# angela000/DQNFlappyBird

Measured on AMD Instinct MI355X. Metric: env steps/sec (whole node) + DQN grad-steps/sec, 80x80x4 batch=32, higher is better.
Workload: dtype f32

## Files before the change

### dqnflappybird_amd/csrc/fb_qnet.hip

```cpp
#include <math.h>
#include <stdlib.h>
#include "fb_common.h"

#ifndef FK_ABL
#define FK_ABL 0
#endif
#ifndef BW_ABL
#define BW_ABL 0
#endif

namespace {

typedef float f32x16 __attribute__((ext_vector_type(16)));

constexpr int OFF_W1 = 0, OFF_B1 = 8192, OFF_W2 = 8224, OFF_B2 = 40992, OFF_W3 = 41056, OFF_B3 = 77920,
              OFF_WF1 = 77984;
constexpr int CONV_PARAMS = OFF_WF1;
#include "fb_head.h"
#include "fb_sampler.h"
#include "fb_gather.h"
constexpr int MAXTB = 256;


struct Slice { const float *params; const uint8_t *states; int s_off, count; const uint16_t *w1s; int fshift; };
// ... 811 lines not shown
                const int Pp = tile * 8 + 2 * g + hl;
                if (Pp < 100) {
                    if (blockIdx.y == 0) { const size_t o = (row * 100 + Pp) * 32 + j; a.p1o[o] = bv; a.amax[o] = (uint8_t)best; }
                    uint16_t *d = reinterpret_cast<uint16_t *>(smem + Pp * 4 + (((j >> 3) + (Pp >> 2)) & 3)) + (j & 7);
                    if constexpr (NS == 3) {
                        const _Float16 hh = (_Float16)bv, ll = (_Float16)((bv - (float)hh) * F16_LO_SCALE);
                        d[0] = __builtin_bit_cast(uint16_t, hh); d[IN_P * 8] = __builtin_bit_cast(uint16_t, ll);
                        bad |= bv >= FB_F16_RANGE;
                    } else d[0] = (uint16_t)f32_to_bf16_rn(bv);
                }
            }
        }
    }
    __syncthreads();
    if (W16 && wave >= 8) { if constexpr (NS == 3) note_overflow(bad, a.ovf); return; }
    if (RING && C23T_EXIT == 2) { if (smem[tid].x == 0x12345u) a.h2[0] = 1.f; return; }
    const int oy = j / 5, ox = j - oy * 5;
    const bool rowok = j < 25;
    f32x16 acc = {0}, acl = {0};
    auto finish = [&](const float *__restrict__ bias, float *__restrict__ out, bool planes) {
#pragma unroll
        for (int r = 0; r < 16; r++) red[((kq * 2 + ct) * 16 + r) * 64 + lane] = NS == 3 ? fmaf(acl[r], F16_LO_UNSCALE, acc[r]) : acc[r];
        __syncthreads();
        const int ctp = wave & 1, q = wave >> 1;
        float v[4];
#pragma unroll
        for (int e = 0; e < 4; e++) {
            v[e] = red[((0 * 2 + ctp) * 16 + 4 * q + e) * 64 + lane];
#pragma unroll
            for (int k = 1; k < 4; k++) v[e] += red[((k * 2 + ctp) * 16 + 4 * q + e) * 64 + lane];
        }
        const int ch = ctp * 32 + 8 * q + 4 * hl;
        const float4 bv = *reinterpret_cast<const float4 *>(bias + ch);
        v[0] = fmaxf(v[0] + bv.x, 0.f); v[1] = fmaxf(v[1] + bv.y, 0.f); v[2] = fmaxf(v[2] + bv.z, 0.f); v[3] = fmaxf(v[3] + bv.w, 0.f);
        if (rowok) *reinterpret_cast<float4 *>(out + (row * 25 + j) * 64 + ch) = make_float4(v[0], v[1], v[2], v[3]);
        if ((planes || a.a3s) && rowok) {
            uint32_t h0, l0, h1, l1, m_;
            if constexpr (NS == 3) { split2x2(v[0], v[1], h0, l0); split2x2(v[2], v[3], h1, l1); bad |= out_of_f16_range(v[0], v[1], v[2], v[3]); }
            else { split3x2(v[0], v[1], h0, m_, l0); split3x2(v[2], v[3], h1, m_, l1); }
            if (planes) {
                uint2 *d = reinterpret_cast<uint2 *>(smem + C2O + j * 8 + ((ctp * 4 + q) ^ ((j >> 1) & 7))) + hl;
                d[0] = make_uint2(h0, h1);
                if (NS == 3) d[2 * C2_P] = make_uint2(l0, l1);
            } else {
                uint16_t *d = a.a3s + (row * 25 + j) * 64 + ch;
                *reinterpret_cast<uint2 *>(d) = make_uint2(h0, h1);
                if (NS == 3) *reinterpret_cast<uint2 *>(d + a.pl3) = make_uint2(l0, l1);
            }
        }
#pragma unroll
        for (int r = 0; r < 16; r++) { acc[r] = 0.f; acl[r] = 0.f; }
    };
#pragma unroll
    for (int c = 0; c < 17; c++) {
        int aidx[2];
        if (c < 8) {
            const int tap = 2 * c + (kq >> 1), iy = 2 * oy + (tap >> 2) - 1, ix = 2 * ox + (tap & 3) - 1, pix = iy * 10 + ix;
            const bool ok = rowok && iy >= 0 && iy < 10 && ix >= 0 && ix < 10;
#pragma unroll
            for (int p = 0; p < NPL; p++) aidx[p] = ok ? p * IN_P + pix * 4 + ((((kq & 1) * 2 + hl) + (pix >> 2)) & 3) : ZOFF;
        } else {
            const int tap = c - 8, ky = tap / 3, iy = oy + ky - 1, ix = ox + (tap - 3 * ky) - 1, pix = iy * 5 + ix;
            const bool ok = rowok && iy >= 0 && iy < 5 && ix >= 0 && ix < 5;
#pragma unroll
            for (int p = 0; p < NPL; p++) aidx[p] = ok ? C2O + p * C2_P + pix * 8 + ((2 * kq + hl) ^ ((pix >> 1) & 7)) : ZOFF;
        }
        uint4 A[NPL];
#pragma unroll
        for (int p = 0; p < NPL; p++) A[p] = smem[aidx[p]];
        const WF W = w0;
        w0 = w1; w1 = w2;
        if (c + 3 < 17) w2 = loadW(c + 3);
        if constexpr (NS == 3) {
            acl = mfma_h(W.v[0], A[1], acl);
            acl = mfma_h(W.v[1], A[0], acl);
            acc = mfma_h(W.v[0], A[0], acc);
        } else acc = mfma_b(W.v[0], A[0], acc);
        if (c == 7) { finish(s.params + OFF_B2, a.h2, true); __syncthreads(); }
    }
    finish(s.params + OFF_B3, a.h3, false);
    if constexpr (NS == 3) note_overflow(bad, a.ovf);
}

constexpr int FC1_SP_KS = 4;
struct Fc1Args { const uint16_t *ain; size_t aplane; const uint16_t *zeros; const uint4 *w; float *hfp; int stot, M, N;
                 const unsigned *pver; unsigned *wver;
                 const uint4 *w2; int m_split;
                 const float *hp_src; float *hp_dst; int hp_n;
                 unsigned long long *set_flag; unsigned long long set_val; };

#ifndef FC1_ABL
#define FC1_ABL 0
#endif
template <int NS>
__global__ __launch_bounds__(256) void fc1_sp_kernel(Fc1Args a) {
    constexpr int NPL = NS == 3 ? 2 : 1, P0 = NS == 3 ? 0 : 2;
    constexpr int ASZ = NPL * 512, BSZ = 4 * NPL * 64, SLOT = ASZ + BSZ;
    __shared__ uint4 smem[3 * SLOT];
    const int lane = threadIdx.x & 63, wave = threadIdx.x >> 6, hl = lane >> 5, j = lane & 31;
    if (a.wver && blockIdx.x == 0 && threadIdx.x == 0) *a.wver = *a.pver;
    if (a.hp_dst) { const int i = blockIdx.x * 256 + threadIdx.x; if (i < a.hp_n) a.hp_dst[i] = a.hp_src[i]; }
    if (a.set_flag && blockIdx.x == 0 && threadIdx.x == 0) fb_flag_store(a.set_flag, a.set_val);
    const int xcd = blockIdx.x & 7, w = blockIdx.x >> 3, nth = a.N >> 7;
    const int ks = xcd & 3, m0 = (w / nth) * 128, n0 = ((xcd >> 2) * nth + w % nth) * 64;
    const int cbase = ks * 12 + (ks < 2 ? ks : 2), count = ks < 2 ? 13 : 12;
    struct St { uint4 a0, a1, a2, a3, b0, b1; };
    const int r0 = min(m0 + (int)(threadIdx.x >> 2), a.M - 1), r1 = min(m0 + 64 + (int)(threadIdx.x >> 2), a.M - 1);
    const uint16_t *pa0 = a.ain + (size_t)r0 * 1600 + (size_t)cbase * 32 + (threadIdx.x & 3) * 8;
    const uint16_t *pa1 = a.ain + (size_t)r1 * 1600 + (size_t)cbase * 32 + (threadIdx.x & 3) * 8;
    auto ldA = [&](int c, int p, int i) { return *reinterpret_cast<const uint4 *>((i ? pa1 : pa0) + p * a.aplane + c * 32); };
    const uint4 *wsel = a.w2 && m0 >= a.m_split ? a.w2 : a.w;
    auto pbq = [&](int q) {
        const int e = wave + 4 * q, k8 = e / NPL, pl = e - k8 * NPL;
        return wsel + ((size_t)(cbase * 4 + k8) * 3 + P0 + pl) * a.N + n0 + lane;
    };
    const uint4 *pb0 = pbq(0), *pb1 = pbq(NPL == 2 ? 1 : 0);
    const size_t bstep = (size_t)12 * a.N;
    auto ldB = [&](int c, int q) {
        (void)c;
        const uint4 *&pb = q == 0 ? pb0 : pb1;
        const uint4 v = *pb;
        pb += bstep;
        return v;
    };
    auto load = [&](int c) {
        St r;
        r.a0 = ldA(c, 0, 0); r.a1 = ldA(c, 0, 1); r.b0 = ldB(c, 0);
        if (NPL == 2) { r.a2 = ldA(c, 1, 0); r.a3 = ldA(c, 1, 1); r.b1 = ldB(c, 1); }
        else { r.a2 = r.a0; r.a3 = r.a0; r.b1 = r.b0; }
        return r;
    };
    auto stA_ = [&](int slot, int p, int i, const uint4 v) {
        const int q = threadIdx.x + 256 * i, row = q >> 2;
        smem[slot * SLOT + p * 512 + row * 4 + ((q + (row >> 2)) & 3)] = v;
    };
    auto store = [&](int slot, const St r) {
        stA_(slot, 0, 0, r.a0); stA_(slot, 0, 1, r.a1);
        uint4 *d = smem + slot * SLOT + ASZ + wave * 64 + lane;
        d[0] = r.b0;
        if (NPL == 2) { stA_(slot, 1, 0, r.a2); stA_(slot, 1, 1, r.a3); d[256] = r.b1; }
    };
    struct Fr { uint4 A[NPL]; uint4 W[2][NPL]; };
    const int row = wave * 32 + j;
    auto readF = [&](int slot, int s) {
        Fr f;
#pragma unroll
        for (int p = 0; p < NPL; p++) {
            f.A[p] = smem[slot * SLOT + p * 512 + row * 4 + ((2 * s + hl + (row >> 2)) & 3)];
#pragma unroll
            for (int ct = 0; ct < 2; ct++) f.W[ct][p] = smem[slot * SLOT + ASZ + ((2 * s + hl) * NPL + p) * 64 + ct * 32 + j];
        }
        return f;
    };
    f32x16 acc[2] = {{0}, {0}}, acl[2] = {{0}, {0}};
    auto compute = [&](const Fr f) {
        if (FC1_ABL == 2) { acc[0][0] += __uint_as_float(f.A[0].x ^ f.W[0][0].y ^ f.W[1][NPL - 1].z ^ f.A[NPL - 1].w); return; }
#pragma unroll
        for (int ct = 0; ct < 2; ct++) {
            if constexpr (NS == 3) {
                acl[ct] = mfma_h(f.A[1], f.W[ct][0], acl[ct]);
                acl[ct] = mfma_h(f.A[0], f.W[ct][1], acl[ct]);
                acc[ct] = mfma_h(f.A[0], f.W[ct][0], acc[ct]);
            } else acc[ct] = mfma_b(f.A[0], f.W[ct][0], acc[ct]);
        }
    };
    St stA = load(0), stB = load(1);
// ... 2817 lines not shown
        FB_CHECK_HIP(hipMemsetD32Async((hipDeviceptr_t)(h->params[which] + h->sac_off.bq1), (int)bits, (size_t)h->A, fb_stream(stream)));
        FB_CHECK_HIP(hipMemsetD32Async((hipDeviceptr_t)(h->params[which] + h->sac_off.bq2), (int)bits, (size_t)h->A, fb_stream(stream)));
    }
    if (is_iqn(h)) {
        const float b = 1.0f;
        uint32_t bits;
        memcpy(&bits, &b, 4);
        FB_CHECK_HIP(hipMemsetD32Async((hipDeviceptr_t)(h->params[which] + h->iqn_off.be), (int)bits, (size_t)h->FC, fb_stream(stream)));
    }
    if (h->noisy)
        hipLaunchKernelGGL(noisy_sigma_init_kernel, dim3((unsigned)((h->n - OFF_WF1 + 255) / 256)), dim3(256), 0, fb_stream(stream), h->mst[which], h->nnet);
    noisy_materialise(h, which, 0, false, fb_stream(stream));
    env_noise_invalidate(h, which, fb_stream(stream));
    c51d_fold(h, which, fb_stream(stream));
    hipLaunchKernelGGL(w1_split_kernel, dim3(32), dim3(256), 0, fb_stream(stream), h->params[which], h->w1s[which], &h->adam->pver[which]);
    resplit_now(h, which, fb_stream(stream));
    FB_LAUNCH_CHECK();
    return FB_OK;
}

extern "C" int fb_qnet_load_params(fb_qnet_t h, int which, const float *flat, void *stream) {
    FB_REQUIRE(h && flat && (which == 0 || which == 1), "fb_qnet_load_params: bad argument");
    FB_CHECK_HIP(hipMemcpyAsync(master(h, which), flat, sizeof(float) * (size_t)h->ntot, hipMemcpyDeviceToDevice, fb_stream(stream)));
    noisy_materialise(h, which, 0, false, fb_stream(stream));
    env_noise_invalidate(h, which, fb_stream(stream));
    hipLaunchKernelGGL(w1_split_kernel, dim3(32), dim3(256), 0, fb_stream(stream), h->params[which], h->w1s[which], &h->adam->pver[which]);
    c51d_fold(h, which, fb_stream(stream));
    resplit_now(h, which, fb_stream(stream));
    FB_LAUNCH_CHECK();
    return FB_OK;
}

extern "C" int fb_qnet_store_params(fb_qnet_t h, int which, float *flat, void *stream) {
    FB_REQUIRE(h && flat && (which == 0 || which == 1), "fb_qnet_store_params: bad argument");
    FB_CHECK_HIP(hipMemcpyAsync(flat, master(h, which), sizeof(float) * (size_t)h->ntot, hipMemcpyDeviceToDevice, fb_stream(stream)));
    return FB_OK;
}

extern "C" int fb_qnet_get_adam_state(fb_qnet_t h, float *m, float *v, float *beta_pows_host) {
    FB_REQUIRE(h, "fb_qnet_get_adam_state: NULL handle");
    FB_CHECK_HIP(hipDeviceSynchronize());
    const size_t nb = sizeof(float) * (size_t)h->ntot;
    if (m) FB_CHECK_HIP(hipMemcpy(m, h->adam_m, nb, hipMemcpyDeviceToDevice));
    if (v) FB_CHECK_HIP(hipMemcpy(v, h->adam_v, nb, hipMemcpyDeviceToDevice));
    if (beta_pows_host) {
        AdamDev a;
        FB_CHECK_HIP(hipMemcpy(&a, h->adam, sizeof(a), hipMemcpyDeviceToHost));
        beta_pows_host[0] = a.b1pow; beta_pows_host[1] = a.b2pow;
    }
    return FB_OK;
}

extern "C" int fb_qnet_set_adam_state(fb_qnet_t h, const float *m, const float *v, const float *beta_pows_host) {
    FB_REQUIRE(h, "fb_qnet_set_adam_state: NULL handle");
    FB_CHECK_HIP(hipDeviceSynchronize());
    const size_t nb = sizeof(float) * (size_t)h->ntot;
    if (m) FB_CHECK_HIP(hipMemcpy(h->adam_m, m, nb, hipMemcpyDeviceToDevice));
    if (v) FB_CHECK_HIP(hipMemcpy(h->adam_v, v, nb, hipMemcpyDeviceToDevice));
    if (beta_pows_host) {
        AdamDev a;
        FB_CHECK_HIP(hipMemcpy(&a, h->adam, sizeof(a), hipMemcpyDeviceToHost));
        a.b1pow = beta_pows_host[0]; a.b2pow = beta_pows_host[1];
        FB_CHECK_HIP(hipMemcpy(h->adam, &a, sizeof(a), hipMemcpyHostToDevice));
    }
    return FB_OK;
}

enum KernelId {
    K_CONV1 = 0, K_CONV2, K_CONV3, K_FC1, K_HEAD, K_LOSS, K_FC1_BWD, K_CONV3_BWD, K_CONV2_BWD, K_CONV1_DW, K_SLAB, K_ADAM,
    K_COUNT
};

struct Plan {
    Slices sl; int ns;
    bool nib;
    uint8_t *actions; float epsilon; uint64_t seed, step;
    bool train;
    int algo, B; const uint8_t *s, *a, *t; const float *r, *isw; double gamma;
    float *loss, *abs_err, *y, *G; bool apply_adam, tick;
    FbHeadRider *head_rider;
    const FbSampleRider *sample_rider;
    const FbRingSrc *ring;
    const FbSplitCtx *split;
    bool any_rows;
    float *probs;
    bool no_head;
    float *ac_value, *ac_logits, *ac_logp; int ac_greedy;
    const float *ac_adv, *ac_ret; float ac_nt;
    bool ppo; const float *ppo_logp, *ppo_value; const long long *ppo_sel;
    bool policy_head; float *sac_q1, *sac_q2; bool sac_temp;
    const float *iqn_tau, *iqn_tau_next; int iqn_m; float *iqn_theta; bool iqn_double, iqn_mu;
};

template <class F> static void with_nsp(int nsp, F f) { if (nsp == 3) f(IntTag<3>{}); else f(IntTag<1>{}); }

template <class T> static void put_seed_words(T &c, uint64_t seed, uint64_t step) {
    c.seed_lo = (uint32_t)seed; c.seed_hi = (uint32_t)(seed >> 32);
    c.step_lo = (uint32_t)step; c.step_hi = (uint32_t)(step >> 32);
}

struct PlanCtx {
    int only; hipStream_t st;
    int maxc, total;
    bool big, trunk, fused, c51, ac, sac, iqn;
    bool state_trunk;
    int nsp, stot; size_t pl1, pl2;
};
static bool runs(const PlanCtx &c, int id) { return c.only < 0 || c.only == id; }

static PlanCtx plan_ctx(const fb_qnet *h, const Plan &p, int only, hipStream_t st) {
    PlanCtx c{only, st, 0, 0};
    for (int z = 0; z < p.ns; z++) { if (p.sl.s[z].count > c.maxc) c.maxc = p.sl.s[z].count; c.total += p.sl.s[z].count; }
    c.big = c.maxc >= 256 || p.any_rows;
    c.nsp = p.train ? h->nsplit_train : h->nsplit;
    c.stot = 3 * h->max_batch; c.pl1 = (size_t)c.stot * 3200; c.pl2 = (size_t)c.stot * 1600;
    c.trunk = p.ring != nullptr;
    c.fused = c.big && p.nib && !p.train && !c.trunk && p.ns == 1;
    c.c51 = h->sup.N > 0;
    c.sac = is_sac(h);
    c.iqn = is_iqn(h);
    c.ac = is_ac(h) || c.sac || c.iqn;
    c.state_trunk = c.ac && p.train && c.big && !c.trunk;
    return c;
}

static C23T trunk_args(fb_qnet *h, const Plan &p, const PlanCtx &c, SplitJob *job) {
    C23T c23t;
    memset(job, 0, sizeof(*job)); memset(&c23t, 0, sizeof(c23t));
    job->FC = h->FC;
    c23t.sl = p.sl; c23t.p1 = h->p1; c23t.h2 = h->h2; c23t.h3 = h->h3; c23t.ovf = &h->adam->ovf;
    for (int z = 0; z < p.ns; z++) {
        const int which = p.sl.s[z].params == h->params[1] ? 1 : 0;
        c23t.w[z] = h->wsp[which] + WSP_W2;
        if (c.only < 0) {
            job->params[which] = h->params[which]; job->wsp[which] = h->wsp[which];
            job->pver[which] = &h->adam->pver[which]; job->wverc[which] = &h->adam->wverc[which];
            c23t.pver[which] = &h->adam->pver[which]; c23t.wverc[which] = &h->adam->wverc[which];
        }
    }
    return c23t;
}

static void ring_trunk(fb_qnet *h, const Plan &p, const PlanCtx &c) {
    SplitJob job;
    C23T c23t = trunk_args(h, p, c, &job);
    if (c.big) { c23t.a3s = h->a3s; c23t.pl3 = c.pl2; }
    c23t.ring = *p.ring; c23t.p1o = h->p1; c23t.amax = h->amax; c23t.ring_fo = h->ring_fo;
    const bool w16 = c.maxc * p.ns <= 256;
    const bool nst = p.ring->c.nstep > 1;
    with_nsp(c.nsp, [&](auto ns) { with_bool(w16, [&](auto w) { with_bool(nst, [&](auto nv) {
        constexpr bool W16 = decltype(w)::value;
        hipLaunchKernelGGL((conv23_t_kernel<decltype(ns)::value, true, W16, decltype(nv)::value>), dim3(c.maxc, p.ns), dim3(W16 ? 1024 : 512), 0, c.st, c23t);
    }); }); });
}

static int large_pass(fb_qnet *h, const Plan &p, const PlanCtx &c, int *z) {
    const int z0 = *z;
    int z1 = z0 + 1;
    while (z1 < p.ns && p.sl.s[z1].params == p.sl.s[z0].params && p.sl.s[z1].count == p.sl.s[z0].count && p.sl.s[z1].s_off == p.sl.s[z1 - 1].s_off + p.sl.s[z1 - 1].count) z1++;
    const Slice s0 = p.sl.s[z0];
    const int which = s0.params == h->params[1] ? 1 : 0, row0 = s0.s_off, rows = s0.count * (z1 - z0);
    const unsigned *pver = c.only < 0 ? &h->adam->pver[which] : nullptr;
    unsigned *wver = c.only < 0 ? &h->adam->wver[which] : nullptr;
    Slice sl = s0;
    sl.count = rows;
    C1Side side;
    memset(&side, 0, sizeof(side));
    if (z1 - z0 > 1) { side.per = s0.count; side.st1 = p.sl.s[z0 + 1].states; side.st2 = z1 - z0 > 2 ? p.sl.s[z0 + 2].states : p.sl.s[z0 + 1].states; }
    if (p.train) { side.p1 = h->p1; side.amax = h->amax; }
    const int t1p = (rows * 100 + 7) / 8, gsp = min(256, (t1p + C1_WAVES - 1) / C1_WAVES);
    if (!c.trunk && !c.state_trunk && !c.fused && runs(c, K_CONV1))
        hipLaunchKernelGGL(conv1_sp_kernel, dim3(gsp), dim3(64 * C1_WAVES), 0, c.st, sl, (const uint8_t *)h->zeros, h->a1s, c.pl1, c.nsp, h->wsp[which], h->FC, pver, (const unsigned *)wver, side, &h->adam->ovf);
    C23Args c23{h->a1s + (size_t)row0 * 3200, c.pl1, h->wsp[which] + WSP_W2, s0.params + OFF_B2, s0.params + OFF_B3, h->a3s + (size_t)row0 * 1600, c.pl2, rows, pver, wver, c.only < 0 ? &h->adam->wverc[which] : nullptr,
                p.train ? h->h2 + (size_t)row0 * 1600 : nullptr, p.train ? h->h3 + (size_t)row0 * 1600 : nullptr,
                s0.states, s0.w1s, s0.params + OFF_B1, s0.params, h->wsp[which], h->FC, &h->adam->ovf};
    Fc1Args af{h->a3s + (size_t)row0 * 1600, c.pl2, h->zeros, h->wsp[which] + WSP_WF1, (c.fused ? h->hf_act : h->hf) + (size_t)row0 * h->FC, c.stot, rows, h->FC,
               c.fused ? pver : nullptr, c.fused ? wver : nullptr, nullptr, 0,
               c.fused ? head_base(h, s0.params) + h->off.bf1 : nullptr, c.fused ? h->hp_act : nullptr, c.fused ? (int)(h->hoff.n - h->off.bf1) : 0,
               c.fused && p.split && c.only < 0 ? &p.split->f->trunk_done : nullptr, p.split ? p.split->seq : 0};
    if (c.trunk && z1 < p.ns && rows % 128 == 0) {
        int z2 = z1 + 1;
        while (z2 < p.ns && p.sl.s[z2].params == p.sl.s[z1].params && p.sl.s[z2].s_off == p.sl.s[z2 - 1].s_off + p.sl.s[z2 - 1].count) z2++;
        const Slice sn = p.sl.s[z1];
        if (z2 == p.ns && sn.s_off == row0 + rows && sn.params != s0.params) {
            int rows2 = 0;
            for (int z = z1; z < z2; z++) rows2 += p.sl.s[z].count;
            af.w2 = h->wsp[sn.params == h->params[1] ? 1 : 0] + WSP_WF1; af.m_split = rows; af.M = rows + rows2;
            z1 = z2;
        }
    }
    *z = z1;
    const dim3 gc((rows + 4) / 5), gf(((af.M + 127) / 128) * (h->FC / 64) * FC1_SP_KS);
    if (c.fused && p.split && c.only < 0 && gc.x > 256 && gc.x % 256 != 0) { c23.round_flag = &p.split->f->last_round; c23.round_val = p.split->seq; c23.round_blk = (int)(gc.x / 256) * 256; }
    with_nsp(c.nsp, [&](auto ns) {
        if (!c.trunk && !c.state_trunk && runs(c, K_CONV2))
            with_bool(c.fused, [&](auto fu) { hipLaunchKernelGGL((conv23_sp_kernel<decltype(ns)::value, 5, decltype(fu)::value>), gc, dim3(512), 0, c.st, c23); });
        if (runs(c, K_FC1)) hipLaunchKernelGGL(fc1_sp_kernel<decltype(ns)::value>, gf, dim3(256), 0, c.st, af);
    });
    if (c.fused && (c.only < 0 || c.only == K_FC1) && (long long)af.hp_n > (long long)gf.x * 256) {
        const size_t done = (size_t)gf.x * 256;
        FB_CHECK_HIP(hipMemcpyAsync(h->hp_act + done, af.hp_src + done, sizeof(float) * ((size_t)af.hp_n - done), hipMemcpyDeviceToDevice, c.st));
    }
    return FB_OK;
}

static void small_trunk(fb_qnet *h, const Plan &p, const PlanCtx &c, bool planes) {
    SplitJob job;
    C23T c23t = trunk_args(h, p, c, &job);
    if (planes) { c23t.a3s = h->a3s; c23t.pl3 = c.pl2; }
    const int t1 = (c.maxc * 100 + 7) / 8;
    if (runs(c, K_CONV1))
        with_bool(p.nib, [&](auto nib) { hipLaunchKernelGGL(conv1_pool_kernel<decltype(nib)::value>, dim3((t1 + 3) / 4, 1, p.ns), dim3(256), 0, c.st, p.sl, h->p1, h->amax, job); });
    if (runs(c, K_CONV2))
        with_nsp(c.nsp, [&](auto ns) { hipLaunchKernelGGL((conv23_t_kernel<decltype(ns)::value, false>), dim3(c.maxc, p.ns), dim3(512), 0, c.st, c23t); });
}

static void small_forward(fb_qnet *h, const Plan &p, const PlanCtx &c) {
    if (!c.trunk) small_trunk(h, p, c, false);
    if (runs(c, K_FC1)) {
        FkArgs fa;
        fa.sl = p.sl; fa.h3 = h->h3; fa.hf = h->hf; fa.qpart = p.train && !c.c51 && !c.ac ? h->qpart : nullptr; fa.FC = h->FC; fa.A = h->A;
        fa.dueling = h->arch == FB_ARCH_DUELING; fa.stot = c.stot; fa.off = h->off;
        hipLaunchKernelGGL(fc1_fk_kernel, dim3((c.maxc + 15) / 16, h->FC / 16, p.ns), dim3(512), 0, c.st, fa);
    }
}

static void launch_dist_head(const fb_qnet *h, const C51HeadArgs &H, int rows, hipStream_t st) {
    with_actions(h->A, [&](auto a) {
        if (is_qr(h)) hipLaunchKernelGGL(qr_head_kernel<decltype(a)::value>, dim3((rows + 3) / 4), dim3(256), 0, st, H);
        else hipLaunchKernelGGL(c51_head_kernel<decltype(a)::value>, dim3((rows + 3) / 4), dim3(256), 0, st, H);
    });
}
// ... 638 lines not shown
    FB_CHECK_HIP(hipMemcpy(v, h->clip_out, sizeof(v), hipMemcpyDeviceToHost));
    if (norm_host) *norm_host = v[0];
    if (scale_host) *scale_host = v[1];
    return FB_OK;
}

static int run_train(fb_qnet *h, Plan &p, void *stream) {
    if (!(p.apply_adam && h->max_grad_norm > 0.f)) return run_plan(h, p, -1, fb_stream(stream));
    p.apply_adam = false;
    const hipEvent_t ev = h->grad_ev;
    h->grad_ev = nullptr;
    int rc = run_plan(h, p, -1, fb_stream(stream));
    h->grad_ev = ev;
    if (rc == FB_OK) rc = fb_qnet_clip_grad(h, h->grad, stream);
    if (rc == FB_OK) rc = fb_qnet_apply_adam(h, h->grad, stream);
    return rc;
}

static int run_train_gathered(fb_qnet *h, Plan &p, int B, void *stream) {
    const int rc = B >= 256 ? fb_qnet_refresh_planes(h, stream) : FB_OK;
    return rc != FB_OK ? rc : run_train(h, p, stream);
}

static void plan_train_tail(fb_qnet *h, Plan &p, float *flat_grad, const FbRingSrc *ring) {
    p.G = flat_grad ? flat_grad : h->grad;
    p.apply_adam = flat_grad == nullptr; p.tick = true;
    p.ring = ring;
    if (ring && ring->c.nstep > 1)
        for (int z = 0; z < p.ns; z++) if (p.sl.s[z].fshift) p.sl.s[z].fshift = ring->c.nstep;
}

static int check_batch(fb_qnet *h, int B, const char *who) {
    FB_REQUIRE(B >= 1 && B <= h->max_batch && B <= MAXTB, "%s: batch %d exceeds min(max_batch, %d)", who, B, MAXTB);
    return FB_OK;
}
static int check_gamma01(double gamma, const char *who) {
    FB_REQUIRE(isfinite(gamma) && gamma >= 0.0 && gamma <= 1.0, "%s: gamma must be in [0, 1] (got %g)", who, gamma);
    return FB_OK;
}

static int train_plan(fb_qnet *h, int algo, int B, const uint8_t *s, const uint8_t *a, const float *r, const uint8_t *s2,
                      const uint8_t *t, const float *isw, double gamma, float *loss, float *abs_err, float *q_target,
                      float *flat_grad, Plan *out, const FbRingSrc *ring = nullptr) {
    FB_REQUIRE(h && a && r && t && loss && (ring || (s && s2)), "fb_qnet_train_step: NULL argument");
    FB_REQUIRE((algo >= 0 && algo <= FB_ALGO_QR_DOUBLE_PER) || is_mdqn_algo(algo) || algo == FB_ALGO_DOUBLE_PER, "fb_qnet_train_step: unknown algo %d", algo);
    FB_REQUIRE(!is_ac(h), "fb_qnet_train_step: an actor-critic net trains through fb_qnet_ac_train_step / fb_ac_train_from_replay only (got algo %d)", algo);
    FB_REQUIRE(!is_sac(h), "fb_qnet_train_step: a SAC net trains through fb_qnet_sac_train_step / fb_sac_train_from_replay only (got algo %d)", algo);
    FB_REQUIRE(!is_iqn(h), "fb_qnet_train_step: an IQN net trains through fb_qnet_iqn_train_step / fb_iqn_train_from_replay only (got algo %d)", algo);
    {
        const bool c51a = is_c51_algo(algo), qra = is_qr_algo(algo);
        FB_REQUIRE(c51a == (h->sup.N > 0 && !is_qr(h)), c51a ? "fb_qnet_train_step: algo %d (C51) needs a C51 net (fb_qnet_create_c51)"
                                                : "fb_qnet_train_step: a C51 net trains with FB_ALGO_C51, FB_ALGO_C51_PER, FB_ALGO_C51_DOUBLE_PER "
                                                  "or FB_ALGO_C51_DOUBLE only (got algo %d)", algo);
        FB_REQUIRE(qra == is_qr(h), qra ? "fb_qnet_train_step: algo %d (QR) needs a QR net (fb_qnet_create_qr)"
                                        : "fb_qnet_train_step: a QR net trains with FB_ALGO_QR, FB_ALGO_QR_DOUBLE, FB_ALGO_QR_PER or "
                                          "FB_ALGO_QR_DOUBLE_PER only (got algo %d)", algo);
    }
    if (const int rb = check_batch(h, B, "fb_qnet_train_step")) return rb;
    FB_REQUIRE(algo != FB_ALGO_PG || (B <= 128 && !ring && gamma >= (double)B), "fb_qnet_train_step: FB_ALGO_PG takes chunks of <= 128 gathered states and gamma = the whole batch's sample count (>= %d)", B);
    FB_REQUIRE(!is_per_algo(algo) || isw, "fb_qnet_train_step: PER needs isw (algo %d)", algo);
    FB_REQUIRE(algo != FB_ALGO_PG || !(h->huber > 0.f), "fb_qnet_train_step: FB_ALGO_PG has no TD error to clip: the net's Huber delta is %g, set it to 0 (fb_qnet_set_huber)", (double)h->huber);
    Plan p; memset(&p, 0, sizeof(p));
    p.ns = 2;
    p.sl.s[0] = Slice{h->params[0], s, 0, B, h->w1s[0], 0};
    if (algo == FB_ALGO_DQN || algo == FB_ALGO_PG) p.sl.s[1] = Slice{h->params[0], s2, B, B, h->w1s[0], 1};
    else if (algo == FB_ALGO_DOUBLE || algo == FB_ALGO_DOUBLE_PER || is_double_c51(algo) || is_double_qr(algo)) { p.sl.s[1] = Slice{h->params[0], s2, B, B, h->w1s[0], 1}; p.sl.s[2] = Slice{h->params[1], s2, 2 * B, B, h->w1s[1], 1}; p.ns = 3; }
    else p.sl.s[1] = Slice{h->params[1], s2, B, B, h->w1s[1], 1};
    if (is_mdqn_algo(algo)) { p.sl.s[2] = Slice{h->params[1], s, 2 * B, B, h->w1s[1], 0}; p.ns = 3; }
    p.sl.rb = h->nsplit_train == 1;
    p.train = true; p.algo = algo; p.B = B; p.s = s; p.a = a; p.r = r; p.t = t; p.isw = isw; p.gamma = gamma;
    p.loss = loss; p.abs_err = abs_err; p.y = q_target;
    plan_train_tail(h, p, flat_grad, ring);
    *out = p;
    return FB_OK;
}

int fb_qnet_train_step_ring(fb_qnet_t h, int algo, int B, const FbRingSrc *ring, const float *isw, double gamma, float *loss, float *abs_err,
                            float *flat_grad, void *stream, const FbSampleRider *rider, const FbSplitCtx *split) {
    FB_REQUIRE(h && ring && ring->idx && ring->a && ring->r && ring->t, "fb_qnet_train_step_ring: NULL argument");
    Plan p;
    int rc = train_plan(h, algo, B, nullptr, ring->a, ring->r, nullptr, ring->t, isw, gamma, loss, abs_err, nullptr, flat_grad, &p, ring);
    if (rc != FB_OK) return rc;
    p.sample_rider = rider;
    p.split = split;
    return run_train(h, p, stream);
}

__global__ void wsplit_both_kernel(const float *__restrict__ p0, const float *__restrict__ p1, uint4 *__restrict__ w0, uint4 *__restrict__ w1, int FC,
                                   const AdamDev *__restrict__ ad) {
    const int n = blockIdx.y;
    if (ad->pver[n] == ad->wver[n]) return;
    wsplit_item(n ? p1 : p0, n ? w1 : w0, FC, blockIdx.x * blockDim.x + threadIdx.x);
}
__global__ void mark_split_both_kernel(AdamDev *ad) {
    const int n = threadIdx.x;
    if (n < 2) { ad->wver[n] = ad->pver[n]; ad->wverc[n] = ad->pver[n]; }
}

int fb_qnet_refresh_planes(fb_qnet_t h, void *stream) {
    FB_REQUIRE(h, "fb_qnet_refresh_planes: NULL handle");
    const int items = wsplit_items(h->FC);
    hipLaunchKernelGGL(wsplit_both_kernel, dim3((items + 255) / 256, 2), dim3(256), 0, fb_stream(stream), h->params[0], h->params[1], h->wsp[0], h->wsp[1],
                       h->FC, (const AdamDev *)h->adam);
    hipLaunchKernelGGL(mark_split_both_kernel, dim3(1), dim3(64), 0, fb_stream(stream), h->adam);
    FB_LAUNCH_CHECK();
    return FB_OK;
}

int fb_qnet_profile_ring(fb_qnet_t h, int kernel, int reps, int algo, int B, const FbRingSrc *ring, float *loss, void *stream) {
    FB_REQUIRE(h && ring && kernel >= 0 && kernel < K_COUNT && reps >= 1, "fb_qnet_profile_ring: bad argument");
    FB_REQUIRE(!is_per_algo(algo), "fb_qnet_profile_ring: uniform memories only");
    Plan p;
    int rc = train_plan(h, algo, B, nullptr, ring->a, ring->r, nullptr, ring->t, nullptr, 0.99, loss, nullptr, nullptr, nullptr, &p, ring);
    if (rc != FB_OK) return rc;
    p.tick = false;
    rc = fb_qnet_refresh_planes(h, stream);
    for (int i = 0; i < reps && rc == FB_OK; i++) rc = run_plan(h, p, kernel, fb_stream(stream));
    return rc;
}

extern "C" int fb_qnet_train_step(fb_qnet_t h, int algo, int B, const uint8_t *s, const uint8_t *a, const float *r,
                                  const uint8_t *s2, const uint8_t *t, const float *isw, double gamma, float *loss,
                                  float *abs_err, float *q_target, float *flat_grad, void *stream) {
    Plan p;
    int rc = train_plan(h, algo, B, s, a, r, s2, t, isw, gamma, loss, abs_err, q_target, flat_grad, &p);
    if (rc != FB_OK) return rc;
    return run_train(h, p, stream);
}

extern "C" int fb_qnet_set_ac(fb_qnet_t h, float value_coef, float entropy_coef) {
    FB_REQUIRE(h, "fb_qnet_set_ac: NULL handle");
    FB_REQUIRE(is_ac(h), "fb_qnet_set_ac: not an actor-critic net (fb_qnet_create_ac)");
    FB_REQUIRE(isfinite(value_coef) && value_coef >= 0.f, "fb_qnet_set_ac: value_coef must be finite and >= 0 (got %g)", (double)value_coef);
    FB_REQUIRE(isfinite(entropy_coef) && entropy_coef >= 0.f, "fb_qnet_set_ac: entropy_coef must be finite and >= 0 (got %g)", (double)entropy_coef);
    h->ac_cv = value_coef; h->ac_ce = entropy_coef;
    return FB_OK;
}

extern "C" int fb_qnet_get_ac(fb_qnet_t h, float *value_coef_host, float *entropy_coef_host) {
    FB_REQUIRE(h, "fb_qnet_get_ac: NULL handle");
    FB_REQUIRE(is_ac(h), "fb_qnet_get_ac: not an actor-critic net (fb_qnet_create_ac)");
    if (value_coef_host) *value_coef_host = h->ac_cv;
    if (entropy_coef_host) *entropy_coef_host = h->ac_ce;
    return FB_OK;
}

extern "C" int fb_qnet_forward_ac(fb_qnet_t h, const uint8_t *states, int batch, float *logits, float *value, void *stream) {
    FB_REQUIRE(h && states && logits && value, "fb_qnet_forward_ac: NULL argument");
    FB_REQUIRE(is_ac(h), "fb_qnet_forward_ac: not an actor-critic net (fb_qnet_create_ac)");
    FB_REQUIRE(rows_ok(h, batch), "fb_qnet_forward_ac: batch %d exceeds 3*max_batch", batch);
    Plan p = forward_plan(h, 0, states, batch);
    p.ac_value = value; p.ac_logits = logits;
    return run_plan(h, p, -1, fb_stream(stream));
}

extern "C" int fb_qnet_act_policy_nib(fb_qnet_t h, const uint8_t *nib_states, int n, uint64_t seed, uint64_t step, int greedy, uint8_t *actions,
                                      float *value, float *logp, float *logits, void *stream) {
    FB_REQUIRE(h && nib_states && (value || is_sac(h)), "fb_qnet_act_policy_nib: NULL argument");
    FB_REQUIRE(is_ac(h) || is_sac(h), "fb_qnet_act_policy_nib: not an actor-critic or SAC net (fb_qnet_create_ac / fb_qnet_create_sac)");
    FB_REQUIRE(actions || !logp, "fb_qnet_act_policy_nib: logp needs actions");
    FB_REQUIRE(rows_ok(h, n), "fb_qnet_act_policy_nib: n %d exceeds 3*max_batch", n);
    Plan p = forward_plan(h, 0, nib_states, n);
    p.nib = true;
    p.actions = actions; p.seed = seed; p.step = step;
    p.ac_value = value; p.ac_logits = logits; p.ac_logp = logp; p.ac_greedy = greedy != 0;
    p.policy_head = true;
    return run_plan(h, p, -1, fb_stream(stream));
}

int fb_qnet_ac_check_train(fb_qnet_t h, int B, int64_t n_total, const char *who) {
    FB_REQUIRE(h && is_ac(h), "%s: not an actor-critic net (fb_qnet_create_ac)", who);
    if (const int rb = check_batch(h, B, who)) return rb;
    FB_REQUIRE(n_total >= (int64_t)B && n_total <= (int64_t)1 << 40, "%s: n_total %lld must be the whole update's sample count (>= the batch %d)", who, (long long)n_total, B);
    return FB_OK;
}

void fb_qnet_ac_scratch(fb_qnet_t h, float **r, uint8_t **t) { *r = h->ac_r; *t = h->ac_t; }
float *fb_qnet_ppo_sum(fb_qnet_t h) { return h->ppo_sum; }

static Plan ac_train_plan(fb_qnet *h, int B, const uint8_t *s, const uint8_t *a, const float *adv, const float *ret, int64_t n_total, float *loss,
                          float *flat_grad, const FbRingSrc *ring) {
    Plan p; memset(&p, 0, sizeof(p));
    p.ns = 1;
    p.sl.s[0] = Slice{h->params[0], s, 0, B, h->w1s[0], 0};
    p.train = true; p.algo = -1; p.B = B; p.s = s; p.a = a; p.ac_adv = adv; p.ac_ret = ret; p.ac_nt = (float)n_total;
    p.loss = loss;
    plan_train_tail(h, p, flat_grad, ring);
    return p;
}

extern "C" int fb_qnet_ac_train_step(fb_qnet_t h, int B, const uint8_t *s, const uint8_t *a, const float *adv, const float *ret, int64_t n_total,
                                     float *loss, float *flat_grad, void *stream) {
    FB_REQUIRE(h && s && a && adv && ret && loss, "fb_qnet_ac_train_step: NULL argument");
    const int rc = fb_qnet_ac_check_train(h, B, n_total, "fb_qnet_ac_train_step");
    if (rc != FB_OK) return rc;
    Plan p = ac_train_plan(h, B, s, a, adv, ret, n_total, loss, flat_grad, nullptr);
    return run_train_gathered(h, p, B, stream);
}
// ... 286 lines not shown
```

Before: 11.20 million.

## Add paired-sample conv2/conv3 trunk kernel reusing weights across two samples

Adds a conv23_t2_kernel in which each 1024-thread block handles two samples. The conv1 weights held in shared memory and the streamed conv2/conv3 weight fragments are each loaded once and then feed MFMAs for both samples, halving the grid and the per-sample weight traffic. It is selected only when the split form is in use, the 16-wave path applies, and the total row count is at least a threshold. In exchange it uses more shared memory and registers per block and has fewer blocks to spread across CUs, so occupancy and parallelism drop.

```diff
diff --git a/dqnflappybird_amd/csrc/fb_qnet.hip b/dqnflappybird_amd/csrc/fb_qnet.hip
--- a/dqnflappybird_amd/csrc/fb_qnet.hip
+++ b/dqnflappybird_amd/csrc/fb_qnet.hip
@@ -917,6 +917,236 @@
     if constexpr (NS == 3) note_overflow(bad, a.ovf);
 }
 
+template <int NS, bool NST>
+__global__ __launch_bounds__(1024) __attribute__((amdgpu_waves_per_eu(4))) void conv23_t2_kernel(C23T a) {
+    constexpr int NPL = NS == 3 ? 2 : 1, P0 = NS == 3 ? 0 : 2;
+    constexpr int IN_P = 400, C2_P = 200, C2O = NPL * IN_P, SP = C2O + NPL * C2_P, ZOFF = 2 * SP, RED = ZOFF + 16;
+    constexpr int NIB_W = FB_NIB_STRIDE / 4;
+    __shared__ uint4 smem[RED + 2 * 2048];
+    __shared__ uint4 lut[256];
+    __shared__ uint32_t nibw[2 * NIB_W];
+    __shared__ unsigned long long fo[2][4];
+    float *red = reinterpret_cast<float *>(smem + RED);
+    const Slice s = a.sl.s[blockIdx.y];
+    if ((int)(2 * blockIdx.x) >= s.count) return;
+    const int tid = threadIdx.x, lane = tid & 63, wave = tid >> 6, hl = lane >> 5, j = lane & 31, ct = wave & 1, kq = wave >> 1;
+    auto sidx = [&](int z) { const int b = 2 * (int)blockIdx.x + z; return b < s.count ? b : s.count - 1; };
+    auto live = [&](int z) { return 2 * (int)blockIdx.x + z < s.count; };
+    auto srow = [&](int z) { return (size_t)s.s_off + sidx(z); };
+    const uint4 *w = a.w[blockIdx.y];
+    if (blockIdx.x == 0 && blockIdx.y == 0 && tid < 2 && a.wverc[tid]) *a.wverc[tid] = *a.pver[tid];
+    struct WF { uint4 v[NPL]; };
+    auto loadW = [&](int c) {
+        WF r;
+#pragma unroll
+        for (int p = 0; p < NPL; p++) r.v[p] = w[((size_t)(8 * c + 2 * kq + hl) * 3 + P0 + p) * 64 + ct * 32 + j];
+        return r;
+    };
+    WF w0 = {}, w1 = {}, w2 = {};
+    if (wave < 8) { w0 = loadW(0); w1 = loadW(1); w2 = loadW(2); }
+    bool bad = false;
+    const uint4 *w1g = reinterpret_cast<const uint4 *>(s.w1s);
+    const int t5 = tid & 511, iz = tid >> 9;
+    const uint4 wc0 = w1g[t5], wc1 = w1g[t5 + 512], wc2 = w1g[t5 + 1024], wc3 = w1g[t5 + 1536];
+    if (wave < 2) {
+        const int z = wave, b = sidx(z);
+        const bool st = blockIdx.y == 0 && live(z);
+        if constexpr (!NST) {
+            if (lane < 4) {
+                long long tt; int e;
+                fb_ring_locate(a.ring.c, a.ring.steps, a.ring.idx[b], lane == 0 && blockIdx.y == 0, tt, e);
+                const unsigned long long o = fb_frame_off(a.ring.c, tt - 3 + s.fshift + lane, e);
+                fo[z][lane] = o;
+                if (st) {
+                    a.ring_fo[b * 4 + lane] = o;
+                    if (lane == 0) {
+                        const size_t mo = (size_t)(tt % a.ring.c.t_f) * a.ring.c.n_envs + e;
+                        a.ring.a[b] = a.ring.c.act[mo]; a.ring.r[b] = a.ring.c.rew[mo]; a.ring.t[b] = a.ring.c.term[mo];
+                    }
+                }
+            }
+        } else {
+            if (lane < FB_NSTEP_MAX) {
+                long long tt; int e;
+                fb_ring_locate(a.ring.c, a.ring.steps, a.ring.idx[b], lane == 0 && blockIdx.y == 0, tt, e);
+                if (lane < 4) {
+                    const unsigned long long o = fb_frame_off(a.ring.c, tt - 3 + s.fshift + lane, e);
+                    fo[z][lane] = o;
+                    if (st) a.ring_fo[b * 4 + lane] = o;
+                }
+                if (blockIdx.y == 0) {
+                    const FbGatherCtx &c = a.ring.c;
+                    const int n = c.nstep, k = lane < n ? lane : 0, s0 = (int)(tt % c.t_f), sk = s0 + k < c.t_f ? s0 + k : s0 + k - c.t_f;
+                    const size_t mo = (size_t)sk * c.n_envs + e;
+                    const float rw = c.rew[mo];
+                    const unsigned long long tmask = __ballot(lane < n && c.term[mo] != 0);
+                    if (lane == 0 && st) a.ring.a[b] = c.act[mo];
+                    const int m = tmask ? __builtin_ctzll(tmask) + 1 : n;
+                    double acc = 0.0, g = 1.0;
+                    for (int q = 0; q < m; q++) { acc += g * (double)__shfl(rw, q); g *= c.gamma; }
+                    if (lane == 0 && st) { a.ring.r[b] = (float)acc; a.ring.t[b] = tmask ? 1 : 0; }
+                }
+            }
+        }
+    }
+    if (tid < 256) lut[tid] = nib_lut_entry(tid);
+    if (tid >= 256 && tid - 256 < 2 * (FB_NIB_STRIDE / 16)) reinterpret_cast<uint4 *>(nibw)[tid - 256] = make_uint4(0u, 0u, 0u, 0u);
+    if (tid < 16) smem[ZOFF + tid] = make_uint4(0u, 0u, 0u, 0u);
+    if (tid < 512) { smem[RED + tid] = wc0; smem[RED + tid + 512] = wc1; smem[RED + tid + 1024] = wc2; smem[RED + tid + 1536] = wc3; }
+    __syncthreads();
+    const uint8_t *fb = reinterpret_cast<const uint8_t *>(a.ring.c.bits);
+    uint32_t fbyte[2][4];
+#pragma unroll
+    for (int r = 0; r < 2; r++) {
+        const int gi = t5 + 512 * r, gc = gi < 800 ? gi : 0;
+#pragma unroll
+        for (int f = 0; f < 4; f++) fbyte[r][f] = fb[fo[iz][f] * 8 + gc];
+    }
+#pragma unroll
+    for (int r = 0; r < 2; r++) {
+        const int gi = t5 + 512 * r, y = gi / 10, g = gi - y * 10;
+        uint32_t o = 0;
+#pragma unroll
+        for (int q = 0; q < 4; q++)
+#pragma unroll
+            for (int f = 0; f < 4; f++) {
+                const uint32_t t2 = (fbyte[r][f] >> (2 * q)) & 3u;
+                o |= ((t2 & 1u) | ((t2 & 2u) << 3)) << (8 * q + f);
+            }
+        if (gi < 800) nibw[iz * NIB_W + (((y + 2) * FB_NIB_PITCH + 4 + 4 * g) >> 2)] = o;
+    }
+    __syncthreads();
+    const uint8_t *nib = reinterpret_cast<const uint8_t *>(nibw);
+    const uint4 *WB = smem + RED + lane;
+    const float bias = s.params[OFF_B1 + j];
+    for (int item = wave; item < 26; item += 16) {
+        const int z = item >= 13 ? 1 : 0, tile = item - 13 * z;
+        const int P = tile * 8 + (j >> 2), pos = j & 3;
+        const int py = P / 10, px = P - py * 10, oy = 2 * py + (pos >> 1), ox = 2 * px + (pos & 1);
+        f32x16 acc = {0}, acl = {0};
+        const uint8_t *base = nib + z * FB_NIB_STRIDE + (4 * (P < 100 ? oy : 0)) * FB_NIB_PITCH + 3 + 2 * (P < 100 ? ox : 0) + hl;
+        unsigned raw[16];
+#pragma unroll
+        for (int c = 0; c < 16; c++) raw[c] = base[(c >> 1) * FB_NIB_PITCH + 2 * (c & 1)];
+#pragma unroll
+        for (int h8 = 0; h8 < 2; h8++) {
+            uint4 A[8];
+#pragma unroll
+            for (int c = 0; c < 8; c++) A[c] = lut[P < 100 ? raw[8 * h8 + c] : 0u];
+#pragma unroll
+            for (int c = 0; c < 8; c++) {
+                acc = mfma_h(A[c], WB[(0 * 16 + 8 * h8 + c) * 64], acc);
+                acl = mfma_h(A[c], WB[(1 * 16 + 8 * h8 + c) * 64], acl);
+            }
+        }
+#pragma unroll
+        for (int r = 0; r < 16; r++) acc[r] = fmaf(acl[r], F16_LO_UNSCALE, acc[r]);
+        const bool st = blockIdx.y == 0 && live(z);
+        const size_t row = srow(z);
+#pragma unroll
+        for (int g = 0; g < 4; g++) {
+            float bv = fmaxf(acc[4 * g] + bias, 0.f);
+            int best = 0;
+#pragma unroll
+            for (int q = 1; q < 4; q++) {
+                const float v = fmaxf(acc[4 * g + q] + bias, 0.f);
+                if (v > bv) { bv = v; best = q; }
+            }
+            const int Pp = tile * 8 + 2 * g + hl;
+            if (Pp < 100) {
+                if (st) { const size_t o = (row * 100 + Pp) * 32 + j; a.p1o[o] = bv; a.amax[o] = (uint8_t)best; }
+                uint16_t *d = reinterpret_cast<uint16_t *>(smem + z * SP + Pp * 4 + (((j >> 3) + (Pp >> 2)) & 3)) + (j & 7);
+                if constexpr (NS == 3) {
+                    const _Float16 hh = (_Float16)bv, ll = (_Float16)((bv - (float)hh) * F16_LO_SCALE);
+                    d[0] = __builtin_bit_cast(uint16_t, hh); d[IN_P * 8] = __builtin_bit_cast(uint16_t, ll);
+                    bad |= bv >= FB_F16_RANGE;
+                } else d[0] = (uint16_t)f32_to_bf16_rn(bv);
+            }
+        }
+    }
+    __syncthreads();
+    if (wave >= 8) { if constexpr (NS == 3) note_overflow(bad, a.ovf); return; }
+    const int oy = j / 5, ox = j - oy * 5;
+    const bool rowok = j < 25;
+    f32x16 acc[2] = {}, acl[2] = {};
+    auto finish = [&](const float *__restrict__ bias, float *__restrict__ out, bool planes) {
+#pragma unroll
+        for (int z = 0; z < 2; z++)
+#pragma unroll
+            for (int r = 0; r < 16; r++) red[z * 8192 + ((kq * 2 + ct) * 16 + r) * 64 + lane] = NS == 3 ? fmaf(acl[z][r], F16_LO_UNSCALE, acc[z][r]) : acc[z][r];
+        __syncthreads();
+        const int ctp = wave & 1, q = wave >> 1, ch = ctp * 32 + 8 * q + 4 * hl;
+        const float4 bv = *reinterpret_cast<const float4 *>(bias + ch);
+#pragma unroll
+        for (int z = 0; z < 2; z++) {
+            float v[4];
+#pragma unroll
+            for (int e = 0; e < 4; e++) {
+                v[e] = red[z * 8192 + ((0 * 2 + ctp) * 16 + 4 * q + e) * 64 + lane];
+#pragma unroll
+                for (int k = 1; k < 4; k++) v[e] += red[z * 8192 + ((k * 2 + ctp) * 16 + 4 * q + e) * 64 + lane];
+            }
+            v[0] = fmaxf(v[0] + bv.x, 0.f); v[1] = fmaxf(v[1] + bv.y, 0.f); v[2] = fmaxf(v[2] + bv.z, 0.f); v[3] = fmaxf(v[3] + bv.w, 0.f);
+            const bool st = rowok && live(z);
+            const size_t row = srow(z);
+            if (st) *reinterpret_cast<float4 *>(out + (row * 25 + j) * 64 + ch) = make_float4(v[0], v[1], v[2], v[3]);
+            if ((planes || a.a3s) && rowok) {
+                uint32_t h0, l0, h1, l1, m_;
+                if constexpr (NS == 3) { split2x2(v[0], v[1], h0, l0); split2x2(v[2], v[3], h1, l1); bad |= out_of_f16_range(v[0], v[1], v[2], v[3]); }
+                else { split3x2(v[0], v[1], h0, m_, l0); split3x2(v[2], v[3], h1, m_, l1); }
+                if (planes) {
+                    uint2 *d = reinterpret_cast<uint2 *>(smem + z * SP + C2O + j * 8 + ((ctp * 4 + q) ^ ((j >> 1) & 7))) + hl;
+                    d[0] = make_uint2(h0, h1);
+                    if (NS == 3) d[2 * C2_P] = make_uint2(l0, l1);
+                } else if (st) {
+                    uint16_t *d = a.a3s + (row * 25 + j) * 64 + ch;
+                    *reinterpret_cast<uint2 *>(d) = make_uint2(h0, h1);
+                    if (NS == 3) *reinterpret_cast<uint2 *>(d + a.pl3) = make_uint2(l0, l1);
+                }
+            }
+        }
+#pragma unroll
+        for (int z = 0; z < 2; z++)
+#pragma unroll
+            for (int r = 0; r < 16; r++) { acc[z][r] = 0.f; acl[z][r] = 0.f; }
+    };
+#pragma unroll
+    for (int c = 0; c < 17; c++) {
+        int aidx[2];
+        bool ok;
+        if (c < 8) {
+            const int tap = 2 * c + (kq >> 1), iy = 2 * oy + (tap >> 2) - 1, ix = 2 * ox + (tap & 3) - 1, pix = iy * 10 + ix;
+            ok = rowok && iy >= 0 && iy < 10 && ix >= 0 && ix < 10;
+#pragma unroll
+            for (int p = 0; p < NPL; p++) aidx[p] = p * IN_P + pix * 4 + ((((kq & 1) * 2 + hl) + (pix >> 2)) & 3);
+        } else {
+            const int tap = c - 8, ky = tap / 3, iy = oy + ky - 1, ix = ox + (tap - 3 * ky) - 1, pix = iy * 5 + ix;
+            ok = rowok && iy >= 0 && iy < 5 && ix >= 0 && ix < 5;
+#pragma unroll
+            for (int p = 0; p < NPL; p++) aidx[p] = C2O + p * C2_P + pix * 8 + ((2 * kq + hl) ^ ((pix >> 1) & 7));
+        }
+        uint4 A[2][NPL];
+#pragma unroll
+        for (int z = 0; z < 2; z++)
+#pragma unroll
+            for (int p = 0; p < NPL; p++) A[z][p] = smem[ok ? z * SP + aidx[p] : ZOFF];
+        const WF W = w0;
+        w0 = w1; w1 = w2;
+        if (c + 3 < 17) w2 = loadW(c + 3);
+#pragma unroll
+        for (int z = 0; z < 2; z++) {
+            if constexpr (NS == 3) {
+                acl[z] = mfma_h(W.v[0], A[z][1], acl[z]);
+                acl[z] = mfma_h(W.v[1], A[z][0], acl[z]);
+                acc[z] = mfma_h(W.v[0], A[z][0], acc[z]);
+            } else acc[z] = mfma_b(W.v[0], A[z][0], acc[z]);
+        }
+        if (c == 7) { finish(s.params + OFF_B2, a.h2, true); __syncthreads(); }
+    }
+    finish(s.params + OFF_B3, a.h3, false);
+    if constexpr (NS == 3) note_overflow(bad, a.ovf);
+}
+
 constexpr int FC1_SP_KS = 4;
 struct Fc1Args { const uint16_t *ain; size_t aplane; const uint16_t *zeros; const uint4 *w; float *hfp; int stot, M, N;
                  const unsigned *pver; unsigned *wver;
@@ -3900,6 +4130,7 @@
     const FbSampleRider *sample_rider;
     const FbRingSrc *ring;
     const FbSplitCtx *split;
+    bool split_form;
     bool any_rows;
     float *probs;
     bool no_head;
@@ -3959,6 +4190,7 @@
     return c23t;
 }
 
+constexpr int TRUNK_PAIR_MIN = 52;
 static void ring_trunk(fb_qnet *h, const Plan &p, const PlanCtx &c) {
     SplitJob job;
     C23T c23t = trunk_args(h, p, c, &job);
@@ -3966,6 +4198,12 @@
     c23t.ring = *p.ring; c23t.p1o = h->p1; c23t.amax = h->amax; c23t.ring_fo = h->ring_fo;
     const bool w16 = c.maxc * p.ns <= 256;
     const bool nst = p.ring->c.nstep > 1;
+    if (w16 && p.split_form && c.total >= TRUNK_PAIR_MIN) {
+        with_nsp(c.nsp, [&](auto ns) { with_bool(nst, [&](auto nv) {
+            hipLaunchKernelGGL((conv23_t2_kernel<decltype(ns)::value, decltype(nv)::value>), dim3((c.maxc + 1) / 2, p.ns), dim3(1024), 0, c.st, c23t);
+        }); });
+        return;
+    }
     with_nsp(c.nsp, [&](auto ns) { with_bool(w16, [&](auto w) { with_bool(nst, [&](auto nv) {
         constexpr bool W16 = decltype(w)::value;
         hipLaunchKernelGGL((conv23_t_kernel<decltype(ns)::value, true, W16, decltype(nv)::value>), dim3(c.maxc, p.ns), dim3(W16 ? 1024 : 512), 0, c.st, c23t);
@@ -4770,7 +5008,7 @@
     int rc = train_plan(h, algo, B, nullptr, ring->a, ring->r, nullptr, ring->t, isw, gamma, loss, abs_err, nullptr, flat_grad, &p, ring);
     if (rc != FB_OK) return rc;
     p.sample_rider = rider;
-    p.split = split;
+    p.split = split; p.split_form = split != nullptr;
     return run_train(h, p, stream);
 }
 
@@ -4802,6 +5040,7 @@
     int rc = train_plan(h, algo, B, nullptr, ring->a, ring->r, nullptr, ring->t, nullptr, 0.99, loss, nullptr, nullptr, nullptr, &p, ring);
     if (rc != FB_OK) return rc;
     p.tick = false;
+    p.split_form = true;
     rc = fb_qnet_refresh_planes(h, stream);
     for (int i = 0; i < reps && rc == FB_OK; i++) rc = run_plan(h, p, kernel, fb_stream(stream));
     return rc;
```

Measured after the change: 11.06 million. 1.2% lower.
